# TrevorS/qwen3-tts-rs

Measured on AMD Instinct MI355X. Metric: acoustic_frames_per_sec, higher is better.
Workload: dtype bf16

## Files before the change

include/q3tts.h:

```cpp
#ifndef Q3TTS_H
#define Q3TTS_H

#include <stddef.h>
#include <stdint.h>

#ifdef __cplusplus
extern "C" {
#endif

#define Q3_ABI_VERSION 1
#define Q3_MAX_BATCH 64

typedef enum q3_status {
    Q3_OK = 0,
    Q3_INVALID_ARG = 1,
    Q3_IO = 2,
    Q3_MISSING_WEIGHT = 3,
    Q3_KV_OVERFLOW = 4,
    Q3_HIP_ERROR = 5,
    Q3_RCCL_ERROR = 6,
    Q3_UNSUPPORTED = 7,
    Q3_OOM = 8
} q3_status;

// ... 209 lines not shown
int         q3_conv_path(int cout, int cin, int L, int k, int dil, int phases, int packed, int has_resid, int planes, int aligned16);
int         q3_resunit_path(int C, int L, int dil, int packed, int ya_is_xa, int planes);
const char* q3_conv_path_name(int code);
typedef struct q3_conv_ex_args {
    int kind, cin, cout, L, k, dil, stride;
    int act, planes, packed, resid_in_place, snake_raw, y2_is_x;
    int y_front, y_elems;
    int* path;
    const float* x; const float* w; const float* b;
    const float* snake_a; const float* snake_b; const float* resid; const float* scale;
    const float* post_a; const float* post_ib;
    const float* w2; const float* b2; const float* mid_a; const float* mid_ib;
    float* y; float* y2;
} q3_conv_ex_args;
q3_status q3_conv_ex(int device, const q3_conv_ex_args* args);
int q3_gemm_path(int M, int N, int K, int epi, int norm, int w2, int planes, int* path);
typedef struct q3_gemm_ex_args {
    int M, N, K, ldx, ldy, ldr, M_alloc;
    int epi, geometry, k_split, sup_m, sup_n;
    float eps;
    int* path;
    const float* x; const uint16_t* w; const uint16_t* w2;
    const float* bias; const float* norm_w; const float* resid;
    float* y;
} q3_gemm_ex_args;
q3_status q3_gemm_ex(int device, const q3_gemm_ex_args* args);
int q3_attn_prefill_path(int nh, int nkv, int use_planes, int halves, int* path);
typedef struct q3_attn_prefill_ex_args {
    int n_seq, rps, base_pos, nh, nkv, max_seq, ld_qkv, ld_out;
    int kernel, halves, use_planes;
// ... 255 lines not shown
```

qwen3_tts_rs_amd/__init__.py:

```python
from .config import Q3Config, qwen3_tts_0_6b, qwen3_tts_1_7b, tiny, tiny_same_width
from .api import (Qwen3TTS, Session, Parked, Batcher, StreamingSession, TextStreamingSession, SynthesisOptions, SynthesisTiming, AudioBuffer, Utterance,
                  Speaker, Language, CODEC_EOS_TOKEN_ID, SAMPLES_PER_FRAME, codes_to_tensor, auto_device,
                  fused_residual_rmsnorm, linear, linear_ex, attn_step, attn_step_ex, kv_pages_to_bf16_ex, gemm_ex, gemm_path, attn_prefill_ex, attn_prefill_path, conv_ex, conv_path, conv_path_name, resunit_path, norm_c, dwconv7, sample, row_move,
                  attn_c_ex, attn_c_path, rope_c_ex, copy_cols_ex, copy_segs_ex, gather_frames_ex, rvq_embed_ex, silu_mul_ex, RefAudio,
                  sample_row, sample_ex, frame_embed_ex, cp_gather_ex, rmsnorm_ex)
from .speaker import SpeakerEncoder, SpeakerEncoderConfig, VoiceClonePrompt, tiny_speaker_config
from .speech_encoder import SpeechEncoder, SpeechEncoderConfig, tiny_speech_config

__all__ = ["Q3Config", "qwen3_tts_0_6b", "qwen3_tts_1_7b", "tiny", "tiny_same_width", "Qwen3TTS", "Session", "Parked", "row_move",
           "StreamingSession", "TextStreamingSession", "SynthesisOptions", "SynthesisTiming", "AudioBuffer", "Utterance", "Speaker", "Language",
           "CODEC_EOS_TOKEN_ID", "SAMPLES_PER_FRAME", "codes_to_tensor", "auto_device", "fused_residual_rmsnorm",
           "linear", "linear_ex", "attn_step", "attn_step_ex", "kv_pages_to_bf16_ex", "gemm_ex", "gemm_path", "attn_prefill_ex", "attn_prefill_path", "conv_ex", "conv_path", "conv_path_name", "resunit_path", "norm_c", "dwconv7", "sample",
           "attn_c_ex", "attn_c_path", "rope_c_ex", "copy_cols_ex", "copy_segs_ex", "gather_frames_ex", "rvq_embed_ex", "silu_mul_ex", "SpeakerEncoder", "SpeakerEncoderConfig", "VoiceClonePrompt", "tiny_speaker_config",
           "SpeechEncoder", "SpeechEncoderConfig", "tiny_speech_config", "RefAudio",
           "sample_row", "sample_ex", "frame_embed_ex", "cp_gather_ex", "rmsnorm_ex"]
```

qwen3_tts_rs_amd/_lib.py:

```python
import ctypes
import os

from .config import CConfig

_HERE = os.path.dirname(os.path.abspath(__file__))
LIB_PATH = os.environ.get("Q3TTS_LIB") or os.path.join(_HERE, "libq3tts.so")

if not os.path.exists(LIB_PATH):
    raise ImportError(
        f"{LIB_PATH} not found: the gfx950 HIP library is not built. Run "
        "`python -c 'import __graft_entry__ as g; g.build()'` (or qwen3_tts_rs_amd/csrc/build.sh).")

lib = ctypes.CDLL(LIB_PATH)


class COptions(ctypes.Structure):
    _fields_ = [
        ("temperature", ctypes.c_double), ("top_p", ctypes.c_double), ("repetition_penalty", ctypes.c_double),
        ("seed", ctypes.c_uint64), ("max_length", ctypes.c_int32), ("top_k", ctypes.c_int32),
        ("eos_token_id", ctypes.c_int32), ("chunk_frames", ctypes.c_int32), ("min_new_tokens", ctypes.c_int32),
        ("has_seed", ctypes.c_int32),
    ]


# ... 238 lines not shown
    "q3_cp_generate": (c_int, [c_void_p, c_void_p, c_void_p, c_void_p, c_void_p]),
    "q3_frame_embed": (c_int, [c_void_p, ctypes.c_uint32, c_void_p, c_void_p, c_void_p]),
    "q3_sample": (c_int, [c_int, c_void_p, c_void_p, c_void_p, c_int, c_int, P(COptions), c_int, c_void_p]),
    "q3_rng_seed": (None, [ctypes.c_uint64, P(ctypes.c_uint64)]),
    "q3_rng_next": (ctypes.c_float, [P(ctypes.c_uint64)]),
    "q3_fused_residual_rmsnorm": (c_int, [c_int, c_int, c_void_p, c_void_p, c_void_p, c_int, c_int, ctypes.c_float, c_void_p, c_void_p]),
    "q3_linear": (c_int, [c_int, c_void_p, c_void_p, c_void_p, c_int, c_int, c_int, c_void_p]),
    "q3_linear_ex": (c_int, [c_int, P(CLinearEx)]),
    "q3_attn_step": (c_int, [c_int, P(CAttnStep)]),
    "q3_attn_step_ex": (c_int, [c_int, P(CAttnStepEx)]),
    "q3_kv_pages_to_bf16_ex": (c_int, [c_int] * 4 + [c_void_p] * 6),
    "q3_conv_path": (c_int, [c_int] * 10),
    "q3_resunit_path": (c_int, [c_int] * 6),
    "q3_conv_path_name": (c_char_p, [c_int]),
    "q3_conv_ex": (c_int, [c_int, P(CConvEx)]),
    "q3_gemm_path": (c_int, [c_int] * 7 + [P(ctypes.c_int32)]),
    "q3_gemm_ex": (c_int, [c_int, P(CGemmEx)]),
    "q3_attn_prefill_path": (c_int, [c_int] * 4 + [P(ctypes.c_int32)]),
    "q3_attn_prefill_ex": (c_int, [c_int, P(CAttnPrefillEx)]),
    "q3_attn_c_path": (c_int, [c_int, c_int]),
    "q3_attn_c_ex": (c_int, [c_int, P(CAttnCEx)]),
    "q3_rope_c_ex": (c_int, [c_int, c_void_p, c_void_p, c_void_p, c_void_p, c_void_p, c_int, c_int, c_int, c_int]),
    "q3_copy_cols_ex": (c_int, [c_int, c_void_p, ctypes.c_size_t, c_void_p, ctypes.c_size_t, c_int, c_int, c_void_p, c_void_p, c_void_p, c_void_p,
                                ctypes.c_size_t, ctypes.c_size_t]),
    "q3_copy_segs_ex": (c_int, [c_int, c_void_p, ctypes.c_size_t, c_void_p, ctypes.c_size_t, c_int, c_void_p]),
    "q3_gather_frames_ex": (c_int, [c_int, c_void_p, ctypes.c_size_t, c_void_p, c_int, c_void_p, ctypes.c_size_t]),
    "q3_rvq_embed_ex": (c_int, [c_int, c_void_p, c_int, c_void_p, c_void_p, c_int, c_int, c_void_p, c_void_p, c_int, c_int]),
    "q3_silu_mul_ex": (c_int, [c_int, c_void_p, c_void_p, c_void_p, ctypes.c_longlong, ctypes.c_longlong]),
    "q3_sample_row": (c_int, [P(COptions), P(CSampleRow)]),
    "q3_sample_ex": (c_int, [c_int, P(CSampleEx)]),
# ... 97 lines not shown
```

qwen3_tts_rs_amd/api.py:

```python
import ctypes
import enum
from dataclasses import dataclass
from typing import List, NamedTuple, Optional, Sequence, Tuple

import numpy as np

from . import _lib
from ._lib import lib, check, COptions, CRequest, CTiming
from .config import Q3Config
from . import synth

MAX_BATCH = 64
CODEC_EOS_TOKEN_ID = 2150
SAMPLES_PER_FRAME = 1920


class Language(enum.Enum):
    Chinese = 2055
    English = 2050
    Japanese = 2058
    Korean = 2064
    German = 2053
    French = 2061
    Russian = 2069
# ... 1950 lines not shown
def silu_mul_ex(g: np.ndarray, u: np.ndarray, y: np.ndarray, device: int = 0) -> np.ndarray:
    g = np.ascontiguousarray(g, dtype=np.float32); u = np.ascontiguousarray(u, dtype=np.float32)
    assert g.ndim == 1 and u.shape == g.shape and y.dtype == np.float32 and y.flags.c_contiguous and y.ndim == 1
    check(lib.q3_silu_mul_ex(device, _vp(g), _vp(u), _vp(y), g.size, y.size))
    return y


def resunit_path(C: int, L: int, dil: int, packed: bool = True, ya_is_xa: bool = False, planes: int = 3) -> int:
    return lib.q3_resunit_path(C, L, dil, int(packed), int(ya_is_xa), planes)


def conv_path_name(code: int) -> str:
    return lib.q3_conv_path_name(code).decode()


def conv_ex(kind: int, x: np.ndarray, w: np.ndarray, *, dil: int = 1, stride: int = 1, b: Optional[np.ndarray] = None, snake=None,
            post=None, mid=None, resid: Optional[np.ndarray] = None, resid_in_place: bool = False, scale: Optional[np.ndarray] = None,
            act: int = 0, planes: int = 3, packed: bool = True, snake_raw: bool = False, w2: Optional[np.ndarray] = None,
            b2: Optional[np.ndarray] = None, y: Optional[np.ndarray] = None, y2: Optional[np.ndarray] = None, y_front: int = 0,
            y2_is_x: bool = False, device: int = 0):
    f = lambda a: np.ascontiguousarray(a, dtype=np.float32)
    x = f(x); w = f(w)
    assert x.ndim == 2 and w.ndim == 3
    cin, L = x.shape
    cout = w.shape[1] if kind == 1 else w.shape[0]
    assert (w.shape[0] if kind == 1 else w.shape[1]) == cin
    a = _lib.CConvEx()
    a.kind, a.cin, a.cout, a.L, a.k, a.dil, a.stride = kind, cin, cout, L, w.shape[2], dil, stride
    a.act, a.planes, a.packed, a.resid_in_place, a.snake_raw, a.y2_is_x = act, planes, int(packed), int(resid_in_place), int(snake_raw), int(y2_is_x)
    n_out = cout * L * (stride if kind == 1 else 1)
# ... 206 lines not shown
```

qwen3_tts_rs_amd/csrc/q3_kernels.h:

```cpp
#pragma once
#include <hip/hip_runtime.h>
#include <stdint.h>

namespace q3 {

constexpr int HEAD_DIM = 128;
constexpr int MAX_SPLITS = 64;
constexpr int PART_STRIDE = HEAD_DIM + 2;
constexpr int KV_PAGE_POS = 128, KV_PAGE_SHIFT = 7, KV_MAX_PAGES = 64;

#ifdef Q3_TRACE
constexpr int TRACE_SLOTS = 8, TRACE_WGS = 512, TRACE_DWGS = 16, TRACE_WAVES = 16;
constexpr int TRACE_NODE = TRACE_SLOTS * (TRACE_WGS + TRACE_DWGS * TRACE_WAVES);
#define Q3_TRACE_FIELD unsigned long long* trace = nullptr;
#if defined(__HIPCC__)
#define Q3T_DECL unsigned long long q3t_[q3::TRACE_SLOTS] = {0, 0, 0, 0, 0, 0, 0, 0};
#define Q3T(i) do { q3t_[i] = (unsigned long long)wall_clock64(); } while (0)
#define Q3T_W(i) do { asm volatile("s_waitcnt vmcnt(0)" ::: "memory"); q3t_[i] = (unsigned long long)wall_clock64(); } while (0)
#define Q3T_K(i, val) do { asm volatile("s_waitcnt lgkmcnt(0)" :: "s"(val) : "memory"); q3t_[i] = (unsigned long long)wall_clock64(); } while (0)
#define Q3T_FLUSH(a, wg) do { if ((a).trace && threadIdx.x == 0 && (int)(wg) < q3::TRACE_WGS) { \
        _Pragma("unroll") for (int q3i_ = 0; q3i_ < q3::TRACE_SLOTS; ++q3i_) (a).trace[(size_t)(wg) * q3::TRACE_SLOTS + q3i_] = q3t_[q3i_]; } \
    if ((a).trace && (threadIdx.x & 63) == 0 && (int)(wg) < q3::TRACE_DWGS && (int)(threadIdx.x >> 6) < q3::TRACE_WAVES) { \
        _Pragma("unroll") for (int q3i_ = 0; q3i_ < q3::TRACE_SLOTS; ++q3i_) \
            (a).trace[(size_t)q3::TRACE_SLOTS * (q3::TRACE_WGS + (wg) * q3::TRACE_WAVES + (threadIdx.x >> 6)) + q3i_] = q3t_[q3i_]; } } while (0)
// ... 221 lines not shown
    CK_NONE = 0,
    CK_OUT1 = 1, CK_OUT1_V4 = 2,
    CK_LIN_SMALL_4W = 3, CK_LIN_SMALL_8W = 4,
    CK_BF16X3_96x128_TM4 = 5,
    CK_BF16X3_4Wx32x128 = 6,
    CK_BF16X3_4Wx32x256 = 7,
    CK_BF16X3_64x128 = 8,
    CK_BF16X3_64x64 = 9,
    CK_BF16X3_128x128 = 10,
    CK_BF16X3_96x128_6W = 11,
    CK_MFMA_F32_64 = 12, CK_MFMA_F32_32 = 13,
    CK_VALU = 14,
    CK_RESUNIT_3W = 15, CK_RESUNIT_6W = 16,
    CK_COUNT = 17
};
enum { CP_KERNEL_MASK = 31, CP_PRE = 32, CP_SEG = 64, CP_CIS128 = 128, CP_NP2 = 256 };
struct ConvPath {
    int kernel = CK_NONE;
    int co_m = 0, t_m = 0, wco = 0, wt = 0;
    bool pre = false, seg = false;
    int cis = 0, np = 0;
    hipError_t refusal = hipSuccess;
};
ConvPath conv_pick(int cout, int cin, int L, int k, int dil, int phases, bool packed, bool has_resid, int planes, bool aligned16,
                   bool transposed = false);
ConvPath resunit_pick(int C, int L, int dil, bool complete, bool ya_is_xa, int planes);
int conv_path_code(const ConvPath& p);
const char* conv_path_name(int code);
hipError_t launch_conv1d(const ConvArgs& a, hipStream_t st, int* path = nullptr);
struct ResUnitArgs {
    const float* xa; float* y; float* ya;
    const void* w1pk; const void* w2pk; const float* b1; const float* b2;
    const float* mid_a; const float* mid_ib; const float* post_a; const float* post_ib;
    int C, L, dil;
    int planes = 3;
};
hipError_t launch_resunit(const ResUnitArgs& r, hipStream_t st, int* path = nullptr);
hipError_t launch_transconv1d_taps(const float* x, const float* wp, const float* b, float* y, int cin, int cout, int L,
                                   int stride, int taps, const float* snake_a, const float* snake_ib, hipStream_t st,
                                   const float* post_a = nullptr, const float* post_ib = nullptr, float* y2 = nullptr,
                                   const void* wpk = nullptr,
                                   int planes = 3, int* path = nullptr);
// ... 122 lines not shown
```

qwen3_tts_rs_amd/csrc/q3_kernels_codec.hip:

```cpp
#include "q3_kernels.h"

#include <math.h>
#include <stdio.h>
#include <stdlib.h>

namespace q3 {

__device__ __forceinline__ float sin_sq(float x) {
    if (fabsf(x) >= 8192.0f) { const float s = sinf(x); return s * s; }
    const float k = rintf(x * 0.31830988618379067154f);
    float r = fmaf(-k, 3.140625f, x);
    r = fmaf(-k, 9.67502593994140625e-4f, r);
    r = fmaf(-k, 1.509957990978376432e-7f, r);
    const float z = r * r;
    float p = fmaf(z, -2.50521083854417188e-8f, 2.75573192239858907e-6f);
    p = fmaf(z, p, -1.98412698412698413e-4f);
    p = fmaf(z, p, 8.33333333333333333e-3f);
    p = fmaf(z, p, -1.66666666666666667e-1f);
    const float s = fmaf(r * z, p, r);
    return s * s;
}
__device__ __forceinline__ float snake_f(float x, float a, float ib) { return add_rn(x, mul_rn(sin_sq(x * a), ib)); }

constexpr int CV_CO = 32, CV_T = 128, CV_CI = 16, CV_MAXK = 7, CV_MAXHALO = 54;
// ... 461 lines not shown
            for (int tm = 0; tm < T_M; ++tm) {
                const int t = t0 + wt * (32 * T_M) + tm * 32 + li;
                if (ook && t < a.L) {
                    float v = acc[cm][tm][reg] + bias;
                    v = conv_act(v, a.act);
                    if (a.scale) v = v * sc;
                    const size_t oi = (size_t)o * a.oL + (size_t)t * a.ostride + ooff;
                    if (a.resid) v = (PRE ? rs[PRE ? tm : 0][reg] : a.resid[oi]) + v;
                    if (a.act == 2) v = fminf(fmaxf(v, -1.0f), 1.0f);
                    if (a.post_a) {
                        const float va = snake_f(v, pa, pib);
                        if (a.y2) { a.y[oi] = v; a.y2[oi] = va; } else a.y[oi] = va;
                    } else {
                        a.y[oi] = v;
                    }
                }
            }
        }
    }
}

struct ResUnitDev {
    const float* xa;
    float* y;
    float* ya;
    const void* w1pk; const void* w2pk;
    const float* b1; const float* b2;
    const float* mid_a; const float* mid_ib;
    const float* post_a; const float* post_ib;
    int C, L, dil;
// ... 334 lines not shown
    return launch_bf16x3_vp<K, CO_M, T_M, WCO, WT, 3>(p, a, phases, st);
}
template <int K>
static hipError_t launch_bf16x3_k(const ConvPath& p, const ConvDev& a, int phases, hipStream_t st) {
    switch (p.kernel) {
        case CK_BF16X3_96x128_TM4: return launch_bf16x3_v<K, 1, 4, 3, 1>(p, a, phases, st);
        case CK_BF16X3_4Wx32x128: return launch_bf16x3_v<K, 1, 4, 4, 1>(p, a, phases, st);
        case CK_BF16X3_4Wx32x256: return launch_bf16x3_v<K, 1, 8, 4, 1>(p, a, phases, st);
        case CK_BF16X3_64x128: return launch_bf16x3_v<K, 1, 2, 2, 2>(p, a, phases, st);
        case CK_BF16X3_64x64: return launch_bf16x3_v<K, 1, 1, 2, 2>(p, a, phases, st);
        case CK_BF16X3_128x128: return launch_bf16x3_v<K, 2, 2, 2, 2>(p, a, phases, st);
        case CK_BF16X3_96x128_6W: return launch_bf16x3_v<K, 1, 2, 3, 2>(p, a, phases, st);
        default: return hipErrorInvalidValue;
    }
}
static int conv_pick_geometry(int K, int cout, int L, int phases, bool has_resid) {
    const long big_tiles = (long)((L + 127) / 128) * (cout / 128) * phases;
    static const int geo = [] { const char* e = getenv("Q3_CONV_TM4"); return e ? atoi(e) : 2; }();
    if (geo && K >= 2 && L >= 4096 && (cout == 192 || cout == 96)) return CK_BF16X3_96x128_TM4;
    if (geo >= 2 && K >= 2 && L >= 4096 && cout % 128 == 0 && big_tiles >= 192) {
        if (geo == 2) return CK_BF16X3_4Wx32x128;
        if (geo == 3) return CK_BF16X3_4Wx32x256;
    }
    if (K == 1 && has_resid && cout % 64 == 0 && cout != 96 && big_tiles >= 192) return CK_BF16X3_64x128;
    {
        static const int pw = [] { const char* e = getenv("Q3_CONV_PW1_GEO"); return e ? atoi(e) : 2; }();
        if (pw && K == 1 && !has_resid && cout % 128 == 0 && big_tiles >= 192 && big_tiles < 1024) {
            if (pw == 1) return CK_BF16X3_64x128;
            return CK_BF16X3_64x64;
        }
// ... 36 lines not shown

ConvPath conv_pick(int cout, int cin, int L, int k, int dil, int phases, bool packed, bool has_resid, int planes, bool aligned16, bool transposed) {
    ConvPath p;
    if (k < 1 || k > CV_MAXK || (k - 1) * dil > CV_MAXHALO || L <= 0 || cout < 1 || cin < 1 || phases < 1) { p.refusal = hipErrorInvalidValue; return p; }
    if (cout == 1 && !transposed) {
        p.kernel = (k == 7 && dil == 1 && L % 4 == 0 && aligned16) ? CK_OUT1_V4 : CK_OUT1;
        return p;
    }
    if (conv_pick_bf16x3(p, cout, cin, L, k, phases, packed, has_resid, conv_planes(planes))) return p;
    if (conv_pick_mfma(p, cout, k)) return p;
    p.kernel = CK_VALU;
    return p;
}

int conv_path_code(const ConvPath& p) {
    return p.kernel | (p.pre ? CP_PRE : 0) | (p.seg ? CP_SEG : 0) | (p.cis == 128 ? CP_CIS128 : 0) | (p.np == 2 ? CP_NP2 : 0);
}
const char* conv_path_name(int code) {
    static const char* const KN[CK_COUNT] = {
        "none", "k_conv_out1", "k_conv_out1_v4", "k_lin_small_bf16x3<4>", "k_lin_small_bf16x3<8>",
        "k_conv_bf16x3<96co x 128t, 3 waves, T_M=4>", "k_conv_bf16x3<4 waves x 32co x 128t>", "k_conv_bf16x3<4 waves x 32co x 256t>",
        "k_conv_bf16x3<64co x 128t>", "k_conv_bf16x3<64co x 64t>", "k_conv_bf16x3<128co x 128t>", "k_conv_bf16x3<96co x 128t, 6 waves>",
        "k_conv1d_mfma<CO_W=2>", "k_conv1d_mfma<CO_W=1>", "k_conv1d", "k_resunit_bf16x3<3>", "k_resunit_bf16x3<6>"};
    static thread_local char buf[96];
    const int k = code & CP_KERNEL_MASK;
    if (code < 0 || k >= CK_COUNT || (code & ~(CP_KERNEL_MASK | CP_PRE | CP_SEG | CP_CIS128 | CP_NP2))) return "invalid";
    snprintf(buf, sizeof buf, "%s%s%s%s%s", KN[k], (code & CP_PRE) ? " PRE" : "", (code & CP_SEG) ? " SEG" : "", (code & CP_CIS128) ? " CIS=128" : "",
             (code & CP_NP2) ? " NP=2" : "");
    return buf;
}

__global__ __launch_bounds__(256) void k_conv_out1(ConvDev a) {
    const int t = blockIdx.x * 256 + threadIdx.x;
    if (t >= a.L) return;
    float acc = 0.0f;
    for (int c = 0; c < a.cin; ++c) {
        const float sa = a.snake_a ? a.snake_a[c] : 0.0f, sib = a.snake_a ? a.snake_ib[c] : 0.0f;
        for (int kk = 0; kk < a.k; ++kk) {
            const int ts = t - (a.k - 1 - kk) * a.dil;
            if (ts < 0) continue;
            float v = a.x[(size_t)c * a.L + ts];
            if (a.snake_a) v = snake_f(v, sa, sib);
            acc = fmaf(a.w[(size_t)c * a.k + kk], v, acc);
// ... 51 lines not shown
                else hipLaunchKernelGGL((k_lin_small_bf16x3<4, 2>), grid, dim3(256), 0, st, a);
            } else {
                if (p.kernel == CK_LIN_SMALL_8W) hipLaunchKernelGGL((k_lin_small_bf16x3<8, 3>), grid, dim3(512), 0, st, a);
                else hipLaunchKernelGGL((k_lin_small_bf16x3<4, 3>), grid, dim3(256), 0, st, a);
            }
            break;
        }
        case CK_MFMA_F32_64:
        case CK_MFMA_F32_32: return launch_conv_mfma(p, a, phases, st);
        case CK_VALU: {
            dim3 grid((a.L + CV_T - 1) / CV_T, (a.cout + CV_CO - 1) / CV_CO, phases);
            hipLaunchKernelGGL(k_conv1d, grid, dim3(256), 0, st, a);
            break;
        }
        default:
            switch (a.k) {
                case 1: return launch_bf16x3_k<1>(p, a, phases, st);
                case 2: return launch_bf16x3_k<2>(p, a, phases, st);
                case 3: return launch_bf16x3_k<3>(p, a, phases, st);
                case 5: return launch_bf16x3_k<5>(p, a, phases, st);
                case 7: return launch_bf16x3_k<7>(p, a, phases, st);
                default: return hipErrorInvalidValue;
            }
    }
    return hipGetLastError();
}

hipError_t launch_conv1d(const ConvArgs& c, hipStream_t st, int* path) {
    const ConvPath p = conv_pick(c.cout, c.cin, c.L, c.k, c.dil, 1, c.wpk != nullptr, c.resid != nullptr, c.planes,
                                 (((uintptr_t)c.x | (uintptr_t)c.y) & 15) == 0, false);
    if (path) *path = conv_path_code(p);
    if (p.kernel == CK_NONE) return p.refusal;
    ConvDev a{};
    a.x = c.x; a.w = c.w; a.b = c.b; a.y = c.y; a.cin = c.cin; a.cout = c.cout; a.L = c.L; a.k = c.k; a.dil = c.dil;
    a.snake_a = c.snake_a; a.snake_ib = c.snake_b; a.resid = c.resid; a.scale = c.scale; a.act = c.act;
    a.ostride = 1; a.ooff = 0; a.oL = c.L; a.w_phase_stride = 0; a.ooff_phase = 0;
    a.post_a = c.post_a; a.post_ib = c.post_ib; a.y2 = c.y2;
    a.wpk = c.wpk; a.wpk_phase_stride = 0; a.planes = conv_planes(c.planes);
    return launch_conv_path(p, a, 1, st);
}

hipError_t launch_transconv1d_taps(const float* x, const float* wp, const float* b, float* y, int cin, int cout, int L,
                                   int stride, int taps, const float* snake_a, const float* snake_ib, hipStream_t st,
                                   const float* post_a, const float* post_ib, float* y2, const void* wpk, int planes, int* path) {
    const ConvPath p = conv_pick(cout, cin, L, taps, 1, stride, wpk != nullptr, false, planes, false, true);
    if (path) *path = conv_path_code(p);
    if (p.kernel == CK_NONE) return p.refusal;
    ConvDev a{};
    a.planes = conv_planes(planes);
    a.wpk = wpk; a.wpk_phase_stride = packed_conv_w_bytes(cout, cin, taps) / 16;
    a.post_a = post_a; a.post_ib = post_ib; a.y2 = y2;
    a.x = x; a.w = wp; a.b = b; a.y = y; a.cin = cin; a.cout = cout; a.L = L; a.k = taps; a.dil = 1;
    a.snake_a = snake_a; a.snake_ib = snake_ib; a.resid = nullptr; a.scale = nullptr; a.act = 0;
    a.ostride = stride; a.ooff = 0; a.oL = L * stride;
    a.w_phase_stride = (size_t)cout * cin * taps; a.ooff_phase = 1;
    return launch_conv_path(p, a, stride, st);
}

void transconv_phase_weights(const float* w, int cin, int cout, int k, int stride, float* out) {
    const int taps = k / stride;
// ... 410 lines not shown
```

qwen3_tts_rs_amd/csrc/q3_testapi.hip:

```cpp
#include "q3_engine.h"

extern "C" q3_status q3_talker_step(q3_session* s, const float* embeds_host, float* hidden_host, float* logits_host) {
    if (!s || !embeds_host) return set_err(Q3_INVALID_ARG, "null argument");
    if (!s->prefilled) return set_err(Q3_INVALID_ARG, "session not prefilled");
    const q3_config& c = s->m->cfg;
    HIPC(hipSetDevice(s->m->device));
    std::vector<int> posv(s->B);
    HIPC(sync_frames(s));
    HIPC(q3_hipMemcpy(posv.data(), s->pos, s->B * 4, hipMemcpyDeviceToHost));
    for (int p : posv) if (p >= s->max_seq) return set_err(Q3_KV_OVERFLOW, "KV cache full (%d)", s->max_seq);
    for (int b = 0; b < s->B; ++b) Q3C(kv_reserve_row(s, b, posv[(size_t)b] + 1));
    HIPC(hipMemcpyAsync(s->tb.X, embeds_host, (size_t)s->B * c.hidden * 4, hipMemcpyHostToDevice, s->stream));
    Q3C(talker_step(s, s->pos, 0, true));
    HIPC(sync_frames(s));
    for (int& p : posv) p += 1;
    HIPC(q3_hipMemcpy(s->pos, posv.data(), s->B * 4, hipMemcpyHostToDevice));
    if (hidden_host) HIPC(q3_hipMemcpy(hidden_host, s->LASTH, (size_t)s->B * c.hidden * 4, hipMemcpyDeviceToHost));
    if (logits_host) HIPC(q3_hipMemcpy(logits_host, s->LOGITS, (size_t)s->B * c.codec_vocab * 4, hipMemcpyDeviceToHost));
    return Q3_OK;
}

extern "C" q3_status q3_cp_generate(q3_session* s, const float* last_hidden_host, const float* sem_embed_host,
                                    uint32_t* codes15_host, float* cp_logits_host) {
    if (!s || !last_hidden_host || !codes15_host) return set_err(Q3_INVALID_ARG, "null argument");
// ... 550 lines not shown
        b.get_row(got, dst_slots[pg], elem, row.data());
        for (int dd = 0; dd < HEAD_DIM; ++dd) { uint32_t u; memcpy(&u, &row[(size_t)dd], 4); dst[at + dd] = (uint16_t)(u >> 16); }
        b.copy_row(b.img, got, dst_slots[pg], elem);
    });
    b.strays(got, stray);
    return Q3_OK;
}

extern "C" int q3_conv_path(int cout, int cin, int L, int k, int dil, int phases, int packed, int has_resid, int planes, int aligned16) {
    return conv_path_code(conv_pick(cout, cin, L, k, dil, phases, packed != 0, has_resid != 0, planes, aligned16 != 0, phases > 1));
}
extern "C" int q3_resunit_path(int C, int L, int dil, int packed, int ya_is_xa, int planes) {
    return conv_path_code(resunit_pick(C, L, dil, packed != 0, ya_is_xa != 0, planes));
}
extern "C" const char* q3_conv_path_name(int code) { return conv_path_name(code); }

extern "C" q3_status q3_conv_ex(int device, const q3_conv_ex_args* p) {
    if (!p || !p->x || !p->w || !p->y) return set_err(Q3_INVALID_ARG, "q3_conv_ex: null argument");
    if (p->path) *p->path = 0;
    const int kind = p->kind, cin = p->cin, cout = p->cout, L = p->L, k = p->k, dil = p->dil;
    if (kind < 0 || kind > 2) return set_err(Q3_INVALID_ARG, "q3_conv_ex: kind 0..2");
    if (cin < 1 || cin > 8192 || cout < 1 || cout > 8192 || L < 1 || L > (1 << 22) || k < 1 || k > 64 || dil < 1 || dil > 64 || p->act < 0 || p->act > 6)
        return set_err(Q3_INVALID_ARG, "q3_conv_ex: bad shape (channels 1..8192, L 1..2^22, k 1..64, dil 1..64, act 0..6)");
    const int stride = kind == 1 ? p->stride : 1;
    if (kind == 1 && (stride < 1 || stride > 16 || k % stride)) return set_err(Q3_INVALID_ARG, "q3_conv_ex: transposed conv needs 1 <= stride <= 16 and k %% stride == 0");
    const int taps = k / stride;
    if (kind == 2 && (cin != cout || k != 7 || !p->w2 || !p->mid_a || !p->mid_ib)) return set_err(Q3_INVALID_ARG, "q3_conv_ex: residual unit needs cin == cout, k == 7, w2 and the middle snake pair");
    if (!p->snake_a != !p->snake_b || !p->post_a != !p->post_ib || !p->mid_a != !p->mid_ib) return set_err(Q3_INVALID_ARG, "q3_conv_ex: half a snake pair");
    if (kind != 0 && (p->resid || p->resid_in_place || p->scale || p->act)) return set_err(Q3_INVALID_ARG, "q3_conv_ex: resid / scale / act belong to kind 0");
    if (kind != 0 && kind != 2 && p->y2_is_x) return set_err(Q3_INVALID_ARG, "q3_conv_ex: y2_is_x belongs to kind 2");
// ... 65 lines not shown
        e = launch_resunit(r, 0, &path);
    }
    if (p->path) *p->path = path;
    if (e == hipErrorInvalidValue || e == hipErrorNotSupported) {
        (void)hipGetLastError();
        return set_err(Q3_UNSUPPORTED, "q3_conv_ex: the launcher refused kind=%d cin=%d cout=%d L=%d k=%d dil=%d stride=%d packed=%d planes=%d (%s)", kind, cin, cout,
                       L, k, dil, stride, p->packed, p->planes, hipGetErrorString(e));
    }
    HIPC(e);
    HIPC(q3_hipDeviceSynchronize());
    HIPC(q3_hipMemcpy(p->y, y, yn * 4, hipMemcpyDeviceToHost));
    if (y2) HIPC(q3_hipMemcpy(p->y2, y2, yn * 4, hipMemcpyDeviceToHost));
    return Q3_OK;
}

static q3_status check_cl_out(const char* who, const void* x, const void* w, const void* y, int C, int L, int y_front, int y_elems) {
    if (!x || !w || !y) return set_err(Q3_INVALID_ARG, "%s: null argument", who);
    if (C < 1 || C > 8192 || L < 1 || L > (1 << 22)) return set_err(Q3_INVALID_ARG, "%s: bad shape (C 1..8192, L 1..2^22)", who);
    if (y_front < 0 || y_elems < 0 || (size_t)y_elems < (size_t)y_front + (size_t)C * L) return set_err(Q3_INVALID_ARG, "%s: y must hold y_front + C * L floats", who);
    return Q3_OK;
}

extern "C" q3_status q3_norm_c(int device, int layernorm, const float* x_host, const float* w_host, const float* b_host, int C, int L, float eps,
                               float* y_host, int y_front, int y_elems) {
    Q3C(check_cl_out("q3_norm_c", x_host, w_host, y_host, C, L, y_front, y_elems));
    if (layernorm && !b_host) return set_err(Q3_INVALID_ARG, "q3_norm_c: LayerNorm needs a bias");
    HIPC(hipSetDevice(device));
    DevPool pool;
    float *x, *w, *b = nullptr, *y;
    const size_t n = (size_t)C * L;
// ... 774 lines not shown
```

Measured before the change: 2836.

## Add wide conv kernel sharing one input tile across 6 or 12 output-channel waves

Adds a new bf16x3 MFMA conv kernel in which one workgroup of 6 or 12 waves covers several 32-channel output groups and phases while sharing a single double-buffered LDS input tile. It is meant to cut repeated input staging and snake/split work across workgroups. By default it is selected only for transposed k=2 convs with cin>=384 and enough workgroups, and it may raise the dynamic LDS limit when needed. A force knob and a conv timing entry point are added for tuning; the larger LDS footprint may lower occupancy.

```diff
diff --git a/include/q3tts.h b/include/q3tts.h
--- a/include/q3tts.h
+++ b/include/q3tts.h
@@ -247,6 +247,8 @@
     float* y; float* y2;
 } q3_conv_ex_args;
 q3_status q3_conv_ex(int device, const q3_conv_ex_args* args);
+int         q3_conv_wide_force(int mode);
+q3_status   q3_conv_time(int device, int kind, int cout, int cin, int L, int k, int dil, int stride, int planes, int reps, float* us, int* path);
 int q3_gemm_path(int M, int N, int K, int epi, int norm, int w2, int planes, int* path);
 typedef struct q3_gemm_ex_args {
     int M, N, K, ldx, ldy, ldr, M_alloc;
diff --git a/qwen3_tts_rs_amd/__init__.py b/qwen3_tts_rs_amd/__init__.py
--- a/qwen3_tts_rs_amd/__init__.py
+++ b/qwen3_tts_rs_amd/__init__.py
@@ -1,7 +1,7 @@
 from .config import Q3Config, qwen3_tts_0_6b, qwen3_tts_1_7b, tiny, tiny_same_width
 from .api import (Qwen3TTS, Session, Parked, Batcher, StreamingSession, TextStreamingSession, SynthesisOptions, SynthesisTiming, AudioBuffer, Utterance,
                   Speaker, Language, CODEC_EOS_TOKEN_ID, SAMPLES_PER_FRAME, codes_to_tensor, auto_device,
-                  fused_residual_rmsnorm, linear, linear_ex, attn_step, attn_step_ex, kv_pages_to_bf16_ex, gemm_ex, gemm_path, attn_prefill_ex, attn_prefill_path, conv_ex, conv_path, conv_path_name, resunit_path, norm_c, dwconv7, sample, row_move,
+                  fused_residual_rmsnorm, linear, linear_ex, attn_step, attn_step_ex, kv_pages_to_bf16_ex, gemm_ex, gemm_path, attn_prefill_ex, attn_prefill_path, conv_ex, conv_wide_force, conv_time, conv_path, conv_path_name, resunit_path, norm_c, dwconv7, sample, row_move,
                   attn_c_ex, attn_c_path, rope_c_ex, copy_cols_ex, copy_segs_ex, gather_frames_ex, rvq_embed_ex, silu_mul_ex, RefAudio,
                   sample_row, sample_ex, frame_embed_ex, cp_gather_ex, rmsnorm_ex)
 from .speaker import SpeakerEncoder, SpeakerEncoderConfig, VoiceClonePrompt, tiny_speaker_config
@@ -10,7 +10,7 @@
 __all__ = ["Q3Config", "qwen3_tts_0_6b", "qwen3_tts_1_7b", "tiny", "tiny_same_width", "Qwen3TTS", "Session", "Parked", "row_move",
            "StreamingSession", "TextStreamingSession", "SynthesisOptions", "SynthesisTiming", "AudioBuffer", "Utterance", "Speaker", "Language",
            "CODEC_EOS_TOKEN_ID", "SAMPLES_PER_FRAME", "codes_to_tensor", "auto_device", "fused_residual_rmsnorm",
-           "linear", "linear_ex", "attn_step", "attn_step_ex", "kv_pages_to_bf16_ex", "gemm_ex", "gemm_path", "attn_prefill_ex", "attn_prefill_path", "conv_ex", "conv_path", "conv_path_name", "resunit_path", "norm_c", "dwconv7", "sample",
+           "linear", "linear_ex", "attn_step", "attn_step_ex", "kv_pages_to_bf16_ex", "gemm_ex", "gemm_path", "attn_prefill_ex", "attn_prefill_path", "conv_ex", "conv_wide_force", "conv_time", "conv_path", "conv_path_name", "resunit_path", "norm_c", "dwconv7", "sample",
            "attn_c_ex", "attn_c_path", "rope_c_ex", "copy_cols_ex", "copy_segs_ex", "gather_frames_ex", "rvq_embed_ex", "silu_mul_ex", "SpeakerEncoder", "SpeakerEncoderConfig", "VoiceClonePrompt", "tiny_speaker_config",
            "SpeechEncoder", "SpeechEncoderConfig", "tiny_speech_config", "RefAudio",
            "sample_row", "sample_ex", "frame_embed_ex", "cp_gather_ex", "rmsnorm_ex"]
diff --git a/qwen3_tts_rs_amd/_lib.py b/qwen3_tts_rs_amd/_lib.py
--- a/qwen3_tts_rs_amd/_lib.py
+++ b/qwen3_tts_rs_amd/_lib.py
@@ -276,6 +276,8 @@
     "q3_resunit_path": (c_int, [c_int] * 6),
     "q3_conv_path_name": (c_char_p, [c_int]),
     "q3_conv_ex": (c_int, [c_int, P(CConvEx)]),
+    "q3_conv_wide_force": (c_int, [c_int]),
+    "q3_conv_time": (c_int, [c_int] * 10 + [P(ctypes.c_float), P(c_int)]),
     "q3_gemm_path": (c_int, [c_int] * 7 + [P(ctypes.c_int32)]),
     "q3_gemm_ex": (c_int, [c_int, P(CGemmEx)]),
     "q3_attn_prefill_path": (c_int, [c_int] * 4 + [P(ctypes.c_int32)]),
diff --git a/qwen3_tts_rs_amd/api.py b/qwen3_tts_rs_amd/api.py
--- a/qwen3_tts_rs_amd/api.py
+++ b/qwen3_tts_rs_amd/api.py
@@ -1988,6 +1988,16 @@
     return lib.q3_conv_path_name(code).decode()
 
 
+def conv_wide_force(mode: int) -> int:
+    return lib.q3_conv_wide_force(mode)
+
+
+def conv_time(kind: int, cout: int, cin: int, L: int, k: int, dil: int = 1, stride: int = 1, planes: int = 3, reps: int = 20, device: int = 0):
+    us = ctypes.c_float(0.0); path = ctypes.c_int32(0)
+    check(lib.q3_conv_time(device, kind, cout, cin, L, k, dil, stride, planes, reps, ctypes.byref(us), ctypes.byref(path)))
+    return us.value, path.value
+
+
 def conv_ex(kind: int, x: np.ndarray, w: np.ndarray, *, dil: int = 1, stride: int = 1, b: Optional[np.ndarray] = None, snake=None,
             post=None, mid=None, resid: Optional[np.ndarray] = None, resid_in_place: bool = False, scale: Optional[np.ndarray] = None,
             act: int = 0, planes: int = 3, packed: bool = True, snake_raw: bool = False, w2: Optional[np.ndarray] = None,
diff --git a/qwen3_tts_rs_amd/csrc/q3_kernels.h b/qwen3_tts_rs_amd/csrc/q3_kernels.h
--- a/qwen3_tts_rs_amd/csrc/q3_kernels.h
+++ b/qwen3_tts_rs_amd/csrc/q3_kernels.h
@@ -259,18 +259,20 @@
     CK_RESUNIT_3W = 15, CK_RESUNIT_6W = 16,
     CK_COUNT = 17
 };
-enum { CP_KERNEL_MASK = 31, CP_PRE = 32, CP_SEG = 64, CP_CIS128 = 128, CP_NP2 = 256 };
+enum { CP_KERNEL_MASK = 31, CP_PRE = 32, CP_SEG = 64, CP_CIS128 = 128, CP_NP2 = 256, CP_WIDE12 = 512, CP_WIDE6 = 1024 };
 struct ConvPath {
     int kernel = CK_NONE;
     int co_m = 0, t_m = 0, wco = 0, wt = 0;
     bool pre = false, seg = false;
     int cis = 0, np = 0;
+    int wide = 0;
     hipError_t refusal = hipSuccess;
 };
 ConvPath conv_pick(int cout, int cin, int L, int k, int dil, int phases, bool packed, bool has_resid, int planes, bool aligned16,
                    bool transposed = false);
 ConvPath resunit_pick(int C, int L, int dil, bool complete, bool ya_is_xa, int planes);
 int conv_path_code(const ConvPath& p);
+int conv_wide_force(int mode);
 const char* conv_path_name(int code);
 hipError_t launch_conv1d(const ConvArgs& a, hipStream_t st, int* path = nullptr);
 struct ResUnitArgs {
diff --git a/qwen3_tts_rs_amd/csrc/q3_kernels_codec.hip b/qwen3_tts_rs_amd/csrc/q3_kernels_codec.hip
--- a/qwen3_tts_rs_amd/csrc/q3_kernels_codec.hip
+++ b/qwen3_tts_rs_amd/csrc/q3_kernels_codec.hip
@@ -1,5 +1,6 @@
 #include "q3_kernels.h"
 
+#include <atomic>
 #include <math.h>
 #include <stdio.h>
 #include <stdlib.h>
@@ -499,6 +500,169 @@
                     } else {
                         a.y[oi] = v;
                     }
+                }
+            }
+        }
+    }
+}
+
+constexpr int WIDE_MAXW = 128 + CV_MAXHALO;
+template <int K, int WCO, int NP>
+__global__ __launch_bounds__(64 * WCO, 3) void k_conv_bf16x3_wide(ConvDev a) {
+    static_assert(K >= 2 && (WCO == 6 || WCO == 12), "tapped convs only: W in (128, 182] is what makes the item count 12");
+    constexpr int NT = 64 * WCO, T_M = 4, T_WG = 128, XPB = XP, NOCT = 4;
+    constexpr int NI = NOCT * 3 / WCO;
+    extern __shared__ __attribute__((aligned(16))) unsigned char smem[];
+    __shared__ float s_prm[4][32 * WCO];
+    const int tid = threadIdx.x, lane = tid & 63;
+    const int wave = __builtin_amdgcn_readfirstlane(tid >> 6);
+    const int li = lane & 31, lk = lane >> 5;
+    const int P = a.phases;
+    int bx, by;
+    {
+        const int per = (a.cout >> 5) * P / WCO, nt = (int)gridDim.x / per, nt8 = nt & ~7, lin = (int)blockIdx.x;
+        int r, tt;
+        if (lin < nt8 * per) { r = lin >> 3; tt = (r / per) * 8 + (lin & 7); r = r % per; }
+        else { const int rem = lin - nt8 * per; tt = nt8 + rem / per; r = rem % per; }
+        bx = tt; by = r;
+    }
+    const int pr = by * WCO + wave;
+    const int co32 = __builtin_amdgcn_readfirstlane(pr / P), bz = __builtin_amdgcn_readfirstlane(pr % P);
+    const int t0 = bx * T_WG, co0 = co32 * 32;
+    if (tid < 32 * WCO) {
+        const int o = ((by * WCO + (tid >> 5)) / P) * 32 + (tid & 31);
+        const bool ok = o < a.cout;
+        s_prm[0][tid] = (a.b && ok) ? a.b[o] : 0.0f;
+        s_prm[1][tid] = (a.scale && ok) ? a.scale[o] : 1.0f;
+        s_prm[2][tid] = (a.post_a && ok) ? a.post_a[o] : 0.0f;
+        s_prm[3][tid] = (a.post_a && ok) ? a.post_ib[o] : 0.0f;
+    }
+    const int halo = (K - 1) * a.dil, W = T_WG + halo;
+    const unsigned plane32 = (unsigned)W * XPB, buf32 = NP * plane32, bfrag = (unsigned)(li * XPB + lk * 16);
+    const cu32x4_t* __restrict__ wpk = reinterpret_cast<const cu32x4_t*>(a.wpk) + (size_t)bz * a.wpk_phase_stride;
+    const int ooff = a.ooff + bz * a.ooff_phase;
+    const int nc16 = a.cin >> 4;
+
+    f32x16_t acc[T_M];
+#pragma unroll
+    for (int j = 0; j < T_M; ++j)
+#pragma unroll
+        for (int r = 0; r < 16; ++r) acc[j][r] = 0.0f;
+
+    const uint64_t wpa = reinterpret_cast<uint64_t>(wpk);
+    const uint64_t wpu = ((uint64_t)(uint32_t)__builtin_amdgcn_readfirstlane((int)(wpa >> 32)) << 32) | (uint32_t)__builtin_amdgcn_readfirstlane((int)wpa);
+    const __amdgpu_buffer_rsrc_t wrs = __builtin_amdgcn_make_buffer_rsrc(reinterpret_cast<void*>(wpu), 0, 0x7fffffff, 0x00020000);
+    auto load_A = [&](cu32x4_t (&A)[NP], int ci0, int kk, int c16l) {
+        const int tile = (co32 * K + kk) * nc16 + (ci0 >> 4) + c16l;
+#pragma unroll
+        for (int pl = 0; pl < NP; ++pl)
+            A[pl] = __builtin_bit_cast(cu32x4_t, __builtin_amdgcn_raw_buffer_load_b128(wrs, lane * 16, (tile * 3 + pl) * 1024, 0));
+    };
+    auto x_load = [&](float (&v)[NI][8], int ci0) {
+#pragma unroll
+        for (int i = 0; i < NI; ++i) {
+            const int c = wave + i * WCO;
+            const int q = c % NOCT, tt = (c / NOCT) * 64 + lane;
+            const int ca = ci0 + q * 8, t = t0 - halo + tt;
+            const int cc = ca < a.cin ? ca : a.cin - 8, tc = t < 0 ? 0 : (t < a.L ? t : a.L - 1);
+            const float* xr = a.x + (size_t)cc * a.L + tc;
+#pragma unroll
+            for (int e = 0; e < 8; ++e) v[i][e] = xr[(size_t)e * a.L];
+        }
+    };
+    auto x_store = [&](float (&v)[NI][8], int ci0, unsigned char* dst) {
+#pragma unroll
+        for (int i = 0; i < NI; ++i) {
+            const int c = wave + i * WCO;
+            const int q = c % NOCT, tt = (c / NOCT) * 64 + lane;
+            const int ca = ci0 + q * 8, t = t0 - halo + tt;
+            const bool ok = tt < W && ca < a.cin && t >= 0 && t < a.L;
+            if (a.snake_a && ca < a.cin) {
+#pragma unroll
+                for (int e = 0; e < 8; ++e) v[i][e] = snake_f(v[i][e], a.snake_a[ca + e], a.snake_ib[ca + e]);
+            }
+#pragma unroll
+            for (int e = 0; e < 8; ++e) v[i][e] = ok ? v[i][e] : 0.0f;
+            if (tt < W) {
+                cu32x4_t h, m, l;
+#pragma unroll
+                for (int e = 0; e < 4; ++e) { uint32_t hh, mm, ll; split3_pair(v[i][2 * e], v[i][2 * e + 1], hh, mm, ll); h[e] = hh; m[e] = mm; l[e] = ll; }
+                unsigned char* row = dst + (unsigned)tt * XPB + q * 16;
+                *reinterpret_cast<cu32x4_t*>(row) = h;
+                *reinterpret_cast<cu32x4_t*>(row + plane32) = m;
+                if constexpr (NP == 3) *reinterpret_cast<cu32x4_t*>(row + 2 * plane32) = l;
+            }
+        }
+    };
+
+    cu32x4_t A[2][NP];
+    float xv[NI][8];
+    x_load(xv, 0);
+    load_A(A[0], 0, 0, 0);
+    x_store(xv, 0, smem);
+    __syncthreads();
+    for (int ci0 = 0, sb = 0; ci0 < a.cin; ci0 += 32, sb ^= 1) {
+        const int n16 = (a.cin - ci0) >= 32 ? 2 : 1;
+        const int n_steps = K * n16, last = n_steps - 1;
+        const int ci_nx = ci0 + 32 < a.cin ? ci0 + 32 : ci0;
+        const unsigned char* cur = smem + sb * buf32;
+        auto do_step = [&](const cu32x4_t (&Af)[NP], int s) {
+            const int kk = s / n16, c16l = s - kk * n16;
+            cu32x4_t B[T_M][NP];
+            const unsigned so = (unsigned)(kk * a.dil * XPB + c16l * 32);
+            const unsigned char* bp0 = cur + (bfrag + so);
+            const unsigned char* bp1 = cur + (bfrag + so + plane32);
+            const unsigned char* bp2 = cur + (bfrag + so + 2 * plane32);
+#pragma unroll
+            for (int tm = 0; tm < T_M; ++tm) {
+                B[tm][0] = *reinterpret_cast<const cu32x4_t*>(bp0 + tm * (32 * XPB));
+                B[tm][1] = *reinterpret_cast<const cu32x4_t*>(bp1 + tm * (32 * XPB));
+                if constexpr (NP == 3) B[tm][2] = *reinterpret_cast<const cu32x4_t*>(bp2 + tm * (32 * XPB));
+            }
+#pragma unroll
+            for (int tm = 0; tm < T_M; ++tm) acc[tm] = mfmaP<NP>(Af, B[tm], acc[tm]);
+        };
+        auto fetch = [&](cu32x4_t (&Ad)[NP], int sp) {
+            const bool nx = sp > last;
+            const int kk = nx ? 0 : sp / n16, c16l = nx ? 0 : sp % n16;
+            __builtin_amdgcn_sched_barrier(0); load_A(Ad, nx ? ci_nx : ci0, kk, c16l); __builtin_amdgcn_sched_barrier(0);
+        };
+        fetch(A[1], 1);
+        x_load(xv, ci0 + 32);
+        __builtin_amdgcn_sched_barrier(0);
+        do_step(A[0], 0);
+        fetch(A[0], 2); do_step(A[1], 1);
+        int st = 2;
+        for (; st + 1 < n_steps; st += 2) {
+            fetch(A[1], st + 1); do_step(A[0], st);
+            fetch(A[0], st + 2); do_step(A[1], st + 1);
+        }
+        if (st < n_steps) do_step(A[0], st);
+        x_store(xv, ci0 + 32, smem + (sb ^ 1) * buf32);
+        __syncthreads();
+    }
+#pragma unroll
+    for (int reg = 0; reg < 16; ++reg) {
+        const int row = (reg & 3) + 8 * (reg >> 2) + 4 * lk;
+        const int o = co0 + row;
+        const bool ook = o < a.cout;
+        const int pi = wave * 32 + row;
+        const float bias = s_prm[0][pi], sc = s_prm[1][pi], pa = s_prm[2][pi], pib = s_prm[3][pi];
+#pragma unroll
+        for (int tm = 0; tm < T_M; ++tm) {
+            const int t = t0 + tm * 32 + li;
+            if (ook && t < a.L) {
+                float v = acc[tm][reg] + bias;
+                v = conv_act(v, a.act);
+                if (a.scale) v = v * sc;
+                const size_t oi = (size_t)o * a.oL + (size_t)t * a.ostride + ooff;
+                if (a.resid) v = a.resid[oi] + v;
+                if (a.act == 2) v = fminf(fmaxf(v, -1.0f), 1.0f);
+                if (a.post_a) {
+                    const float va = snake_f(v, pa, pib);
+                    if (a.y2) { a.y[oi] = v; a.y2[oi] = va; } else a.y[oi] = va;
+                } else {
+                    a.y[oi] = v;
                 }
             }
         }
@@ -863,6 +1027,68 @@
         default: return hipErrorInvalidValue;
     }
 }
+static std::atomic<int> g_conv_wide_force{-1};
+int conv_wide_force(int mode) { return g_conv_wide_force.exchange(mode); }
+template <int K, int WCO, int NP>
+static bool conv_wide_lds_ok() {
+    static std::atomic<int> state[64];
+    int dev = 0;
+    if (hipGetDevice(&dev) != hipSuccess || dev < 0 || dev >= 64) { (void)hipGetLastError(); return false; }
+    int s = state[dev].load();
+    if (!s) {
+        const hipError_t e = hipFuncSetAttribute(reinterpret_cast<const void*>(&k_conv_bf16x3_wide<K, WCO, NP>), hipFuncAttributeMaxDynamicSharedMemorySize,
+                                                 2 * NP * WIDE_MAXW * XP);
+        if (e != hipSuccess) (void)hipGetLastError();
+        s = e == hipSuccess ? 1 : 2;
+        state[dev].store(s);
+    }
+    return s == 1;
+}
+static bool conv_wide_lds_ok(int k, int wco, int np) {
+#define Q3_WL(K_, W_, N_) if (k == K_ && wco == W_ && np == N_) return conv_wide_lds_ok<K_, W_, N_>()
+    Q3_WL(7, 12, 3); Q3_WL(7, 6, 3); Q3_WL(2, 12, 3); Q3_WL(2, 6, 3); Q3_WL(7, 12, 2); Q3_WL(7, 6, 2); Q3_WL(2, 12, 2); Q3_WL(2, 6, 2);
+#undef Q3_WL
+    return false;
+}
+static int conv_wide_fit(const ConvPath& p, int cout, int cin, int k, int phases) {
+    if (p.kernel < CK_BF16X3_96x128_TM4 || p.kernel > CK_BF16X3_96x128_6W || p.cis != 32 || p.pre || p.seg) return 0;
+    if ((k != 7 && !(k == 2 && phases > 1)) || cin % 16 || cin < 32 || cout % 32) return 0;
+    const int pairs = (cout / 32) * phases;
+    return pairs % 12 == 0 ? 12 : (pairs % 6 == 0 ? 6 : 0);
+}
+static bool conv_wide_measured_gain(int cout, int cin, int L, int k, int phases, int wco) {
+    const long wgs = (long)((L + 127) / 128) * ((cout / 32) * phases / wco);
+    return k == 2 && phases > 1 && cin >= 384 && wgs >= 256;
+}
+static void conv_pick_wide(ConvPath& p, int cout, int cin, int L, int k, int dil, int phases) {
+    static const bool off = getenv("Q3_CONV_NO_WIDE") != nullptr;
+    const int force = g_conv_wide_force.load();
+    if (off || force == 0) return;
+    const int wco = conv_wide_fit(p, cout, cin, k, phases);
+    if (!wco) return;
+    if (force < 0) {
+        if (p.np != 3 || !conv_wide_measured_gain(cout, cin, L, k, phases, wco)) return;
+    }
+    const size_t lds = (size_t)2 * p.np * (128 + (k - 1) * dil) * XP;
+    if (lds > 65536 && (force == 2 || !conv_wide_lds_ok(k, wco, p.np))) return;
+    p.wide = wco;
+}
+
+template <int K, int WCO, int NP>
+static hipError_t launch_bf16x3_wide_i(const ConvDev& a, int phases, hipStream_t st) {
+    const size_t lds = (size_t)2 * NP * (128 + (K - 1) * a.dil) * XP;
+    const int per = (a.cout / 32) * phases / WCO;
+    ConvDev ap = a; ap.phases = phases;
+    hipLaunchKernelGGL((k_conv_bf16x3_wide<K, WCO, NP>), dim3(((a.L + 127) / 128) * per), dim3(64 * WCO), lds, st, ap);
+    return hipGetLastError();
+}
+static hipError_t launch_bf16x3_wide(const ConvPath& p, const ConvDev& a, int phases, hipStream_t st) {
+    if ((a.cout / 32) * phases % p.wide || a.cin % 16 || (a.k - 1) * a.dil > CV_MAXHALO) return hipErrorInvalidValue;
+#define Q3_WL(K_, W_, N_) if (a.k == K_ && p.wide == W_ && p.np == N_) return launch_bf16x3_wide_i<K_, W_, N_>(a, phases, st)
+    Q3_WL(7, 12, 3); Q3_WL(7, 6, 3); Q3_WL(2, 12, 3); Q3_WL(2, 6, 3); Q3_WL(7, 12, 2); Q3_WL(7, 6, 2); Q3_WL(2, 12, 2); Q3_WL(2, 6, 2);
+#undef Q3_WL
+    return hipErrorInvalidValue;
+}
 static int conv_pick_geometry(int K, int cout, int L, int phases, bool has_resid) {
     const long big_tiles = (long)((L + 127) / 128) * (cout / 128) * phases;
     static const int geo = [] { const char* e = getenv("Q3_CONV_TM4"); return e ? atoi(e) : 2; }();
@@ -929,7 +1155,8 @@
 }
 
 int conv_path_code(const ConvPath& p) {
-    return p.kernel | (p.pre ? CP_PRE : 0) | (p.seg ? CP_SEG : 0) | (p.cis == 128 ? CP_CIS128 : 0) | (p.np == 2 ? CP_NP2 : 0);
+    return p.kernel | (p.pre ? CP_PRE : 0) | (p.seg ? CP_SEG : 0) | (p.cis == 128 ? CP_CIS128 : 0) | (p.np == 2 ? CP_NP2 : 0) |
+           (p.wide == 12 ? CP_WIDE12 : p.wide == 6 ? CP_WIDE6 : 0);
 }
 const char* conv_path_name(int code) {
     static const char* const KN[CK_COUNT] = {
@@ -939,9 +1166,9 @@
         "k_conv1d_mfma<CO_W=2>", "k_conv1d_mfma<CO_W=1>", "k_conv1d", "k_resunit_bf16x3<3>", "k_resunit_bf16x3<6>"};
     static thread_local char buf[96];
     const int k = code & CP_KERNEL_MASK;
-    if (code < 0 || k >= CK_COUNT || (code & ~(CP_KERNEL_MASK | CP_PRE | CP_SEG | CP_CIS128 | CP_NP2))) return "invalid";
-    snprintf(buf, sizeof buf, "%s%s%s%s%s", KN[k], (code & CP_PRE) ? " PRE" : "", (code & CP_SEG) ? " SEG" : "", (code & CP_CIS128) ? " CIS=128" : "",
-             (code & CP_NP2) ? " NP=2" : "");
+    if (code < 0 || k >= CK_COUNT || (code & ~(CP_KERNEL_MASK | CP_PRE | CP_SEG | CP_CIS128 | CP_NP2 | CP_WIDE12 | CP_WIDE6))) return "invalid";
+    snprintf(buf, sizeof buf, "%s%s%s%s%s%s", KN[k], (code & CP_PRE) ? " PRE" : "", (code & CP_SEG) ? " SEG" : "", (code & CP_CIS128) ? " CIS=128" : "",
+             (code & CP_NP2) ? " NP=2" : "", (code & CP_WIDE12) ? " WIDE=12" : (code & CP_WIDE6) ? " WIDE=6" : "");
     return buf;
 }
 
@@ -1023,6 +1250,7 @@
             break;
         }
         default:
+            if (p.wide) return launch_bf16x3_wide(p, a, phases, st);
             switch (a.k) {
                 case 1: return launch_bf16x3_k<1>(p, a, phases, st);
                 case 2: return launch_bf16x3_k<2>(p, a, phases, st);
@@ -1036,8 +1264,9 @@
 }
 
 hipError_t launch_conv1d(const ConvArgs& c, hipStream_t st, int* path) {
-    const ConvPath p = conv_pick(c.cout, c.cin, c.L, c.k, c.dil, 1, c.wpk != nullptr, c.resid != nullptr, c.planes,
-                                 (((uintptr_t)c.x | (uintptr_t)c.y) & 15) == 0, false);
+    ConvPath p = conv_pick(c.cout, c.cin, c.L, c.k, c.dil, 1, c.wpk != nullptr, c.resid != nullptr, c.planes,
+                           (((uintptr_t)c.x | (uintptr_t)c.y) & 15) == 0, false);
+    conv_pick_wide(p, c.cout, c.cin, c.L, c.k, c.dil, 1);
     if (path) *path = conv_path_code(p);
     if (p.kernel == CK_NONE) return p.refusal;
     ConvDev a{};
@@ -1052,7 +1281,8 @@
 hipError_t launch_transconv1d_taps(const float* x, const float* wp, const float* b, float* y, int cin, int cout, int L,
                                    int stride, int taps, const float* snake_a, const float* snake_ib, hipStream_t st,
                                    const float* post_a, const float* post_ib, float* y2, const void* wpk, int planes, int* path) {
-    const ConvPath p = conv_pick(cout, cin, L, taps, 1, stride, wpk != nullptr, false, planes, false, true);
+    ConvPath p = conv_pick(cout, cin, L, taps, 1, stride, wpk != nullptr, false, planes, false, true);
+    conv_pick_wide(p, cout, cin, L, taps, 1, stride);
     if (path) *path = conv_path_code(p);
     if (p.kernel == CK_NONE) return p.refusal;
     ConvDev a{};
diff --git a/qwen3_tts_rs_amd/csrc/q3_testapi.hip b/qwen3_tts_rs_amd/csrc/q3_testapi.hip
--- a/qwen3_tts_rs_amd/csrc/q3_testapi.hip
+++ b/qwen3_tts_rs_amd/csrc/q3_testapi.hip
@@ -588,6 +588,7 @@
     return conv_path_code(resunit_pick(C, L, dil, packed != 0, ya_is_xa != 0, planes));
 }
 extern "C" const char* q3_conv_path_name(int code) { return conv_path_name(code); }
+extern "C" int q3_conv_wide_force(int mode) { return conv_wide_force(mode < -1 || mode > 2 ? -1 : mode); }
 
 extern "C" q3_status q3_conv_ex(int device, const q3_conv_ex_args* p) {
     if (!p || !p->x || !p->w || !p->y) return set_err(Q3_INVALID_ARG, "q3_conv_ex: null argument");
@@ -683,6 +684,56 @@
     return Q3_OK;
 }
 
+extern "C" q3_status q3_conv_time(int device, int kind, int cout, int cin, int L, int k, int dil, int stride, int planes, int reps, float* us, int* path) {
+    if (!us || kind < 0 || kind > 1 || reps < 1 || reps > 1000) return set_err(Q3_INVALID_ARG, "q3_conv_time: kind 0..1, reps 1..1000, us");
+    if (cin < 16 || cin > 8192 || cin % 16 || cout < 32 || cout > 8192 || cout % 32 || L < 1 || L > (1 << 22) || k < 1 || k > 64 || dil < 1 || dil > 64)
+        return set_err(Q3_INVALID_ARG, "q3_conv_time: bad shape (cin %% 16, cout %% 32, L 1..2^22)");
+    if (kind == 0) stride = 1;
+    if (stride < 1 || stride > 16 || k % stride) return set_err(Q3_INVALID_ARG, "q3_conv_time: 1 <= stride <= 16, k %% stride == 0");
+    const int taps = k / stride;
+    const size_t xn = (size_t)cin * L, wn = (size_t)cout * cin * k, yn = (size_t)cout * L * stride;
+    HIPC(hipSetDevice(device));
+    DevPool pool;
+    float *x, *w, *b, *pa, *pb, *y;
+    HIPC(pool.alloc(&x, xn)); HIPC(pool.alloc(&w, wn)); HIPC(pool.alloc(&b, (size_t)cout)); HIPC(pool.alloc(&pa, (size_t)cout)); HIPC(pool.alloc(&pb, (size_t)cout));
+    HIPC(pool.alloc(&y, yn));
+    uint64_t s = 0x9E3779B97F4A7C15ull;
+    auto fill = [&](float* d, size_t n, float scale) -> q3_status {
+        std::vector<float> h(n);
+        for (size_t i = 0; i < n; ++i) { s = s * 6364136223846793005ull + 1442695040888963407ull; h[i] = scale * ((float)(int32_t)(s >> 32) * (1.0f / 2147483648.0f)); }
+        HIPC(q3_hipMemcpy(d, h.data(), n * 4, hipMemcpyHostToDevice));
+        return Q3_OK;
+    };
+    Q3C(fill(x, xn, 1.0f)); Q3C(fill(w, wn, 1.0f / sqrtf((float)cin * taps))); Q3C(fill(b, (size_t)cout, 1.0f)); Q3C(fill(pa, (size_t)cout, 1.0f)); Q3C(fill(pb, (size_t)cout, 1.0f));
+    const size_t per = packed_conv_w_bytes(cout, cin, taps);
+    char* wpk; HIPC(pool.alloc(&wpk, per * (size_t)stride));
+    for (int ph = 0; ph < stride; ++ph) HIPC(launch_pack_conv_w(w + (size_t)ph * cout * cin * taps, wpk + (size_t)ph * per, cout, cin, taps, 0));
+    HIPC(q3_hipDeviceSynchronize());
+    int pth = 0;
+    auto launch = [&]() -> hipError_t {
+        if (kind == 1) return launch_transconv1d_taps(x, w, b, y, cin, cout, L, stride, taps, nullptr, nullptr, 0, pa, pb, nullptr, wpk, planes, &pth);
+        ConvArgs a;
+        a.x = x; a.w = w; a.b = b; a.y = y; a.cin = cin; a.cout = cout; a.L = L; a.k = k; a.dil = dil; a.post_a = pa; a.post_ib = pb; a.wpk = wpk; a.planes = planes;
+        return launch_conv1d(a, 0, &pth);
+    };
+    hipEvent_t e0, e1;
+    HIPC(hipEventCreate(&e0)); HIPC(hipEventCreate(&e1));
+    hipError_t e = hipSuccess;
+    for (int i = 0; i < 3 && e == hipSuccess; ++i) e = launch();
+    if (e == hipSuccess) e = hipEventRecord(e0, 0);
+    for (int i = 0; i < reps && e == hipSuccess; ++i) e = launch();
+    if (e == hipSuccess) e = hipEventRecord(e1, 0);
+    if (e == hipSuccess) e = hipEventSynchronize(e1);
+    float ms = 0.0f;
+    if (e == hipSuccess) e = hipEventElapsedTime(&ms, e0, e1);
+    (void)hipEventDestroy(e0); (void)hipEventDestroy(e1);
+    if (path) *path = pth;
+    if (e == hipErrorInvalidValue || e == hipErrorNotSupported) { (void)hipGetLastError(); return set_err(Q3_UNSUPPORTED, "q3_conv_time: the launcher refused the shape (%s)", hipGetErrorString(e)); }
+    HIPC(e);
+    *us = ms * 1000.0f / (float)reps;
+    return Q3_OK;
+}
+
 static q3_status check_cl_out(const char* who, const void* x, const void* w, const void* y, int C, int L, int y_front, int y_elems) {
     if (!x || !w || !y) return set_err(Q3_INVALID_ARG, "%s: null argument", who);
     if (C < 1 || C > 8192 || L < 1 || L > (1 << 22)) return set_err(Q3_INVALID_ARG, "%s: bad shape (C 1..8192, L 1..2^22)", who);
```

After: 2842, median of 6. Within noise of the previous version (+0.2%).
